# DIAGNijmegen/bodyct-dram-emph-subtype

Hardware: AMD Instinct MI355X
Metric: CT volumes/sec (train step, 1x128x256x256) (higher is better)
Workload: dtype f32; 1 GPU; BASELINE configs[1]: resnet18segcls train step (fwd+loss+bwd+Adam), batch 2/GPU, 1x128x256x256, fp32, inputs resident in HBM; global_batch=2, parallelism=dp1, hip_graph=False, streams=2

## Files before the change

### bodyct-dram-emph-subtype_amd/csrc/bn.hip

```cpp
#include <stdlib.h>
#include <atomic>
#include "common.h"

namespace {

template <typename T>
__global__ void reduce_partials_kernel(const T* __restrict__ partial, double* __restrict__ out, int nparts,
                                       int RC, double tail, int has_tail) {
  __shared__ double sm[256];
  const int col = blockIdx.x * 64 + (threadIdx.x & 63);
  const int lane4 = threadIdx.x >> 6;
  const int S = gridDim.y, sidx = blockIdx.y;
  double s = 0.0;
  if (col < RC)
    for (int p = sidx + S * lane4; p < nparts; p += 4 * S) s += (double)partial[(long)p * RC + col];
  sm[threadIdx.x] = s;
  __syncthreads();
  if (lane4 == 0 && col < RC)
    out[(long)sidx * RC + col] = sm[threadIdx.x] + sm[threadIdx.x + 64] + sm[threadIdx.x + 128] + sm[threadIdx.x + 192];
  if (has_tail && blockIdx.x == 0 && blockIdx.y == 0 && threadIdx.x == 0) out[RC] = tail;
}

__global__ void bn_finalize_kernel(const double* __restrict__ sums, double count_host,
                                   const double* __restrict__ count_dev, const float* __restrict__ gamma,
// ... 25 lines not shown
  scale[c] = sc;
  shift[c] = (float)((double)beta[c] - m * (double)gamma[c] * is);
}

struct FoldFinalize {
  double count;
  const float* gamma; const float* beta; float* rmean; float* rvar;
  float momentum, eps; int update;
  float* mean; float* invstd; float* scale; float* shift;
};
constexpr int FOLD_XMAX = 512;

__global__ __launch_bounds__(1024) void fold_partials_kernel(const float* __restrict__ partial, double* scratch,
                                                             double* __restrict__ sums, float* __restrict__ sums_f32,
                                                             float* __restrict__ f32_row1, const int nparts, const int RC,
                                                             const double tail,
                                                             const int has_tail, unsigned* __restrict__ ticket,
                                                             const FoldFinalize ff) {
  __shared__ double sm[1024];
  __shared__ double tot[64];
  __shared__ unsigned s_ticket;
  const int t64 = threadIdx.x & 63, lane4 = threadIdx.x >> 6;
  const int C = RC >> 1;
  const int col = ff.gamma ? (t64 >> 5) * C + blockIdx.x * 32 + (t64 & 31) : blockIdx.x * 64 + t64;
  const bool live = ff.gamma ? (blockIdx.x * 32 + (t64 & 31) < C) : (col < RC);
  const int S = gridDim.y, sidx = blockIdx.y;
  double s = 0.0;
  if (live) {
    const int step = 16 * S;
    int p = sidx + S * lane4;
    for (; p + 7 * step < nparts; p += 8 * step) {
      float v[8];
#pragma unroll
      for (int j = 0; j < 8; ++j) v[j] = partial[(long)(p + j * step) * RC + col];
#pragma unroll
      for (int j = 0; j < 8; ++j) s += (double)v[j];
    }
    for (; p < nparts; p += step) s += (double)partial[(long)p * RC + col];
  }
  sm[threadIdx.x] = s;
  __syncthreads();
  double total = 0.0;
  if (lane4 == 0) {
#pragma unroll
    for (int j = 0; j < 16; ++j) total += sm[t64 + 64 * j];
  }
  if (S > 1) {
    if (lane4 == 0 && live) scratch[(long)sidx * RC + col] = total;
    __threadfence();
    __syncthreads();
    if (threadIdx.x == 0) s_ticket = atomicAdd(&ticket[blockIdx.x], 1u);
    __syncthreads();
    if (s_ticket != (unsigned)S - 1) return;
    __threadfence();
    if (lane4 == 0 && live) {
      total = 0.0;
      int k = 0;
      for (; k + 8 <= S; k += 8) {
        double v[8];
#pragma unroll
        for (int j = 0; j < 8; ++j)
          v[j] = __hip_atomic_load(scratch + (long)(k + j) * RC + col, __ATOMIC_RELAXED, __HIP_MEMORY_SCOPE_AGENT);
#pragma unroll
        for (int j = 0; j < 8; ++j) total += v[j];
      }
      for (; k < S; ++k)
        total += __hip_atomic_load(scratch + (long)k * RC + col, __ATOMIC_RELAXED, __HIP_MEMORY_SCOPE_AGENT);
    }
  }
  if (lane4 == 0 && live) {
    sums[col] = total;
    if (sums_f32) {
      if (f32_row1 && col >= C) f32_row1[col - C] = (float)total;
      else sums_f32[col] = (float)total;
    }
  }
  if (has_tail && blockIdx.x == 0 && threadIdx.x == 0) sums[RC] = tail;
  if (!ff.gamma) return;
  if (lane4 == 0) tot[t64] = total;
  __syncthreads();
  const int c = blockIdx.x * 32 + threadIdx.x;
  if (threadIdx.x < 32 && c < C) {
    const double m = tot[threadIdx.x] / ff.count;
    double v = tot[32 + threadIdx.x] / ff.count - m * m;
    if (v < 0.0) v = 0.0;
    if (ff.update) {
      const double unb = ff.count > 1.0 ? v * (ff.count / (ff.count - 1.0)) : v;
      ff.rmean[c] = (float)((1.0 - (double)ff.momentum) * (double)ff.rmean[c] + (double)ff.momentum * m);
      ff.rvar[c] = (float)((1.0 - (double)ff.momentum) * (double)ff.rvar[c] + (double)ff.momentum * unb);
    }
    const double is = 1.0 / sqrt(v + (double)ff.eps);
    ff.mean[c] = (float)m;
    ff.invstd[c] = (float)is;
    ff.scale[c] = (float)((double)ff.gamma[c] * is);
    ff.shift[c] = (float)((double)ff.beta[c] - m * (double)ff.gamma[c] * is);
  }
}

template <int RES, typename T>
__global__ void bn_apply_kernel(const T* __restrict__ y, const float* __restrict__ scale,
                                const float* __restrict__ shift, const T* __restrict__ res, int Cr, int rs,
                                T* __restrict__ z, int D, int H, int W, int C, long total4, int relu) {
  const int Q = C >> 2;
  for (long i = blockIdx.x * (long)blockDim.x + threadIdx.x; i < total4; i += (long)gridDim.x * blockDim.x) {
    const int q = (int)(i % Q);
    const float4 sc = *reinterpret_cast<const float4*>(scale + 4 * q);
// ... 359 lines not shown
  }
  const long t0 = n4 * 4;
  for (long i = t0 + blockIdx.x * (long)blockDim.x + threadIdx.x; i < n; i += (long)gridDim.x * blockDim.x)
    os[i] = as[i] + bs[i];
}

inline int ew_grid(long total4) {
  long b = (total4 + 255) / 256;
  return (int)(b > 4096 ? 4096 : (b < 1 ? 1 : b));
}

inline int rows_per_block(long long rows) {
  long long rpb = (rows + 1023) / 1024;
  if (rpb < 64) rpb = 64;
  return (int)rpb;
}

}

extern "C" int dram_reduce_partials_stages(int nparts) {
  if (nparts <= 64) return 1;
  int s = (nparts + 31) / 32;
  return s > 64 ? 64 : s;
}

extern "C" int dram_reduce_partials(const float* partial, double* sums, double* scratch, int nparts, int R, int C,
                                    double tail, int has_tail, dram_stream_t stream) {
  if (!partial || !sums || nparts < 1 || R < 1 || C < 1) return DRAM_ERR_BAD_ARG;
  const int RC = R * C;
  const int S = dram_reduce_partials_stages(nparts);
  hipStream_t st = (hipStream_t)stream;
  DramProf prof(DRAM_FAM_BN, 0, 0.0, 4.0 * (double)nparts * RC + 8.0 * RC, st);
  if (S == 1) {
    hipLaunchKernelGGL((reduce_partials_kernel<float>), dim3((RC + 63) / 64, 1), dim3(256), 0, st, partial, sums,
                       nparts, RC, tail, has_tail);
  } else {
    if (!scratch) return DRAM_ERR_WORKSPACE;
    hipLaunchKernelGGL((reduce_partials_kernel<float>), dim3((RC + 63) / 64, S), dim3(256), 0, st, partial, scratch,
                       nparts, RC, 0.0, 0);
    DRAM_LAUNCH_CHECK();
    hipLaunchKernelGGL((reduce_partials_kernel<double>), dim3((RC + 63) / 64, 1), dim3(256), 0, st,
                       (const double*)scratch, sums, S, RC, tail, has_tail);
  }
  DRAM_LAUNCH_CHECK();
  return DRAM_OK;
}

extern "C" int dram_fold_partials_stages(int nparts) {
  if (nparts <= 1024) return 1;
  const int s = (nparts + 511) / 512;
  return s > 64 ? 64 : s;
}

static int fold_launch(const float* partial, double* sums, double* scratch, float* sums_f32, float* f32_row1, int nparts,
                       int RC, double tail, int has_tail, const FoldFinalize& ff, hipStream_t st) {
  const int S = dram_fold_partials_stages(nparts);
  const int gx = ff.gamma ? (RC / 2 + 31) / 32 : (RC + 63) / 64;
  if (S > 1 && gx > FOLD_XMAX) return DRAM_ERR_UNSUPPORTED;
  unsigned* ticket = nullptr;
  if (S > 1) {
    ticket = reinterpret_cast<unsigned*>(scratch + (long)S * RC);
    const hipError_t e = hipMemsetAsync(ticket, 0, sizeof(unsigned) * gx, st);
    if (e != hipSuccess) return (int)e;
  }
  DramProf prof(DRAM_FAM_BN, 0, 0.0, 4.0 * (double)nparts * RC + 8.0 * RC, st);
  hipLaunchKernelGGL(fold_partials_kernel, dim3(gx, S), dim3(1024), 0, st, partial, scratch, sums, sums_f32, f32_row1,
                     nparts, RC, tail, has_tail, ticket, ff);
  DRAM_LAUNCH_CHECK();
  return DRAM_OK;
}

extern "C" int dram_fold_partials(const float* partial, double* sums, double* scratch, float* sums_f32, float* f32_row1,
                                  int nparts, int R, int C, double tail, int has_tail, dram_stream_t stream) {
  if (!partial || !sums || !scratch || nparts < 1 || R < 1 || C < 1) return DRAM_ERR_BAD_ARG;
  if (f32_row1 && (R != 2 || !sums_f32)) return DRAM_ERR_BAD_ARG;
  FoldFinalize ff{};
  return fold_launch(partial, sums, scratch, sums_f32, f32_row1, nparts, R * C, tail, has_tail, ff, (hipStream_t)stream);
}

extern "C" int dram_bn_fold_finalize(const float* partial, double* sums, double* scratch, int nparts, int C, double count,
                                     const float* gamma, const float* beta, float* running_mean, float* running_var,
                                     float momentum, float eps, int update_running, float* mean, float* invstd,
                                     float* scale, float* shift, dram_stream_t stream) {
  if (!partial || !sums || !scratch || nparts < 1 || C < 1 || count <= 0.0) return DRAM_ERR_BAD_ARG;
  if (!gamma || !beta || !mean || !invstd || !scale || !shift) return DRAM_ERR_BAD_ARG;
  if (update_running && (!running_mean || !running_var)) return DRAM_ERR_BAD_ARG;
  FoldFinalize ff{count, gamma, beta, running_mean, running_var, momentum, eps, update_running, mean, invstd, scale, shift};
  return fold_launch(partial, sums, scratch, nullptr, nullptr, nparts, 2 * C, 0.0, 0, ff, (hipStream_t)stream);
}

extern "C" int dram_bn_finalize(const double* sums, double count, const double* count_dev, const float* gamma,
                                const float* beta,
                                float* running_mean, float* running_var, float momentum, float eps,
                                int update_running, float* mean, float* invstd, float* scale, float* shift, int C,
                                dram_stream_t stream) {
  if (!gamma || !beta || !mean || !invstd || !scale || !shift || C < 1) return DRAM_ERR_BAD_ARG;
  if (!sums && (!running_mean || !running_var)) return DRAM_ERR_BAD_ARG;
  if (sums && !count_dev && count <= 0.0) return DRAM_ERR_BAD_ARG;
  if (update_running && (!running_mean || !running_var)) return DRAM_ERR_BAD_ARG;
  DramProf prof(DRAM_FAM_BN, 1, 0.0, 4.0 * 10.0 * C, (hipStream_t)stream);
  hipLaunchKernelGGL(bn_finalize_kernel, dim3((C + 255) / 256), dim3(256), 0, (hipStream_t)stream, sums, count,
                     count_dev, gamma, beta, running_mean, running_var, momentum, eps, update_running, mean, invstd, scale,
                     shift, C);
  DRAM_LAUNCH_CHECK();
  return DRAM_OK;
}

template <typename T>
static int bn_apply_impl(const T* y, const float* scale, const float* shift, const T* residual, int Dr, int Hr, int Wr,
                         int Cr, int rs, T* z, int B, int D, int H, int W, int C, int relu, dram_stream_t stream) {
  if (!y || !scale || !shift || !z || B < 1 || D < 1 || H < 1 || W < 1 || C < 4 || (C & 3)) return DRAM_ERR_BAD_ARG;
  const long total4 = (long)B * D * H * W * (C >> 2);
  hipStream_t s = (hipStream_t)stream;
  const int grid = ew_blocks(total4, 256);
  const double res_frac = !residual ? 0.0 : ((double)Cr / C) / ((double)rs * rs * rs);
  DramProf prof(DRAM_FAM_BN, 2, 0.0, 4.0 * sizeof(T) * (double)total4 * (2.0 + res_frac), s);
  const int Q = C >> 2;
  const bool identity = residual && rs == 1 && Cr == C && Dr == D && Hr == H && Wr == W;
  if ((!residual || identity) && 256 % Q == 0) {
    const int g1 = ew_blocks(total4, 1024);
#define BN_SHOT_(RES_, NT_) hipLaunchKernelGGL((bn_apply_shot_kernel<RES_, T, NT_>), dim3(g1), dim3(256), 0, s, y, scale, \
                                               shift, residual, z, Q, total4, relu)
    const bool nt = ew_stream(sizeof(T) * 4 * total4);
    if (!residual) { if (nt) BN_SHOT_(0, true); else BN_SHOT_(0, false); }
    else           { if (nt) BN_SHOT_(1, true); else BN_SHOT_(1, false); }
#undef BN_SHOT_
  } else if (!residual) {
    hipLaunchKernelGGL((bn_apply_kernel<0, T>), dim3(grid), dim3(256), 0, s, y, scale, shift, (const T*)nullptr, 0,
                       1, z, D, H, W, C, total4, relu);
  } else if (identity) {
    hipLaunchKernelGGL((bn_apply_kernel<1, T>), dim3(grid), dim3(256), 0, s, y, scale, shift, residual,
                       Cr, 1, z, D, H, W, C, total4, relu);
  } else {
    if ((Cr & 3) || Cr < 4 || Cr > C || rs < 1) return DRAM_ERR_BAD_ARG;
    if ((D - 1) * rs >= Dr || (H - 1) * rs >= Hr || (W - 1) * rs >= Wr) return DRAM_ERR_BAD_ARG;
    hipLaunchKernelGGL((bn_apply_shortcut_a_kernel<T>), dim3(grid), dim3(256), 0, s, y, scale, shift,
                       residual, Dr, Hr, Wr, Cr, rs, z, D, H, W, C, total4, relu);
  }
  DRAM_LAUNCH_CHECK();
  return DRAM_OK;
}
// ... 151 lines not shown
```

### bodyct-dram-emph-subtype_amd/csrc/pool_up.hip

```cpp
#include <stdlib.h>
#include <initializer_list>
#include "common.h"

namespace {

inline int ew_grid(long total) { return ew_blocks(total, 256); }

template <typename T, int VW>
__global__ void maxpool_fwd_kernel(const T* __restrict__ x, T* __restrict__ y,
                                   uint8_t* __restrict__ amax, int D, int H, int W, int C, int Do, int Ho, int Wo,
                                   long total) {
  const int Q = C / VW;
  for (long i = blockIdx.x * (long)blockDim.x + threadIdx.x; i < total; i += (long)gridDim.x * blockDim.x) {
    const int q = (int)(i % Q);
    long v = i / Q;
    const int xo = (int)(v % Wo); v /= Wo;
    const int yo = (int)(v % Ho); v /= Ho;
    const int zo = (int)(v % Do);
    const long b = v / Do;
    fvec<VW> m;
    int am[VW];
#pragma unroll
    for (int k = 0; k < VW; ++k) { m.v[k] = -INFINITY; am[k] = 0; }
    bool first = true;
// ... 258 lines not shown
      o.v[k] += w_ * t.x; o.v[k + 1] += w_ * t.y; o.v[k + 2] += w_ * t.z; o.v[k + 3] += w_ * t.w; \
    }                                                                                        \
  }
      UPT_ACC(za, ya, xa, wz0 * wy0 * wx0) UPT_ACC(za, ya, xc, wz0 * wy0 * wx1)
      UPT_ACC(za, yc, xa, wz0 * wy1 * wx0) UPT_ACC(za, yc, xc, wz0 * wy1 * wx1)
      UPT_ACC(zc, ya, xa, wz1 * wy0 * wx0) UPT_ACC(zc, ya, xc, wz1 * wy0 * wx1)
      UPT_ACC(zc, yc, xa, wz1 * wy1 * wx0) UPT_ACC(zc, yc, xc, wz1 * wy1 * wx1)
#undef UPT_ACC
      const long vox = ((b * Do + zo) * Ho + yo) * (long)Wo + xo;
      stv<T, VW>(cat, vox * Ct + cb + VW * q, o);
    }
  }
  for (int e = tid; e < 512 * Qk; e += 256) {
    const int qq = e % Qk, v = e / Qk;
    const int zo = z0 + (v >> 6), yo = y0 + ((v >> 3) & 7), xo = x0 + (v & 7);
    if (zo >= Do || yo >= Ho || xo >= Wo) continue;
    const long vox = ((b * Do + zo) * Ho + yo) * (long)Wo + xo;
    stv<T, VW>(cat, vox * Ct + Cu + VW * qq,
               ldv<T, VW>(skip, (((b * Dk + zo + oz) * Hk + yo + oy) * Wk + xo + ox) * (long)Ck + VW * qq));
  }
}

__device__ __forceinline__ void dst_range(int s, float scale, int out, int& lo, int& hi) {
  if (scale <= 0.f) { lo = 0; hi = out - 1; return; }
  const float inv = 1.f / scale;
  lo = (int)floorf((float)(s - 1) * inv) - 1;
  hi = (int)ceilf((float)(s + 1) * inv) + 1;
  if (lo < 0) lo = 0;
  if (hi > out - 1) hi = out - 1;
}

struct UpAxis {
  int lo;
  float w[6];
};
__device__ __forceinline__ UpAxis up_axis(int s, float scale, int in, int out) {
  UpAxis t;
  int lo = scale > 0.f ? (int)floorf((float)(s - 1) / scale) - 1 : 0;
  if (lo < 0) lo = 0;
  t.lo = lo;
#pragma unroll
  for (int j = 0; j < 6; ++j) {
    const int d = lo + j;
    int a0, a1;
    float u0, u1;
    lin_src(d, scale, in, a0, a1, u0, u1);
    const float w = (a0 == s ? u0 : 0.f) + (a1 == s ? u1 : 0.f);
    t.w[j] = d < out ? w : 0.f;
  }
  return t;
}

template <typename T, int VW>
__global__ void upcat_bwd_src_kernel(const T* __restrict__ dcat, T* __restrict__ dsrc, int Ds, int Hs, int Ws,
                                     int Cu, int Ct, float sz, float sy, float sx, long total) {
  const int Do = 2 * Ds, Ho = 2 * Hs, Wo = 2 * Ws;
  const int Qu = Cu / VW;
  for (long i = blockIdx.x * (long)blockDim.x + threadIdx.x; i < total; i += (long)gridDim.x * blockDim.x) {
    const int q = (int)(i % Qu);
    long v = i / Qu;
    const int xs = (int)(v % Ws); v /= Ws;
    const int ys = (int)(v % Hs); v /= Hs;
    const int zs = (int)(v % Ds);
    const long b = v / Ds;
    const UpAxis tz = up_axis(zs, sz, Ds, Do), ty = up_axis(ys, sy, Hs, Ho), tx = up_axis(xs, sx, Ws, Wo);
    fvec<VW> acc;
#pragma unroll
    for (int k = 0; k < VW; ++k) acc.v[k] = 0.f;
#pragma unroll
    for (int jz = 0; jz < 6; ++jz) {
      if (tz.w[jz] == 0.f) continue;
#pragma unroll
      for (int jy = 0; jy < 6; ++jy) {
        const float wzy = tz.w[jz] * ty.w[jy];
        if (wzy == 0.f) continue;
        const T* row = dcat + (((b * Do + tz.lo + jz) * Ho + ty.lo + jy) * (long)Wo + tx.lo) * (long)Ct + VW * q;
        fvec<VW> g[6];
#pragma unroll
        for (int jx = 0; jx < 6; ++jx)
          g[jx] = ldv<T, VW>(row, (long)(tx.w[jx] != 0.f ? jx : 0) * Ct);
#pragma unroll
        for (int jx = 0; jx < 6; ++jx) {
          const float w_ = wzy * tx.w[jx];
#pragma unroll
          for (int k = 0; k < VW; ++k) acc.v[k] = __builtin_fmaf(w_, g[jx].v[k], acc.v[k]);
        }
      }
    }
    stv<T, VW>(dsrc, VW * i, acc);
  }
}

template <typename T, int VW>
__global__ void upcat_bwd_skip_kernel(const T* __restrict__ dcat, T* __restrict__ dskip, int Do, int Ho,
                                      int Wo, int Cu, int Dk, int Hk, int Wk, int Ck, int oz, int oy, int ox,
                                      long total) {
  const int Qk = Ck / VW;
  const int Ct = Cu + Ck;
  for (long i = blockIdx.x * (long)blockDim.x + threadIdx.x; i < total; i += (long)gridDim.x * blockDim.x) {
    const int q = (int)(i % Qk);
    long v = i / Qk;
    const int xk = (int)(v % Wk); v /= Wk;
    const int yk = (int)(v % Hk); v /= Hk;
    const int zk = (int)(v % Dk);
    const long b = v / Dk;
    const int zo = zk - oz, yo = yk - oy, xo = xk - ox;
    fvec<VW> o;
#pragma unroll
    for (int k = 0; k < VW; ++k) o.v[k] = 0.f;
    if (zo >= 0 && zo < Do && yo >= 0 && yo < Ho && xo >= 0 && xo < Wo)
      o = ldv<T, VW>(dcat, (((b * Do + zo) * Ho + yo) * Wo + xo) * (long)Ct + Cu + VW * q);
    stv<T, VW>(dskip, VW * i, o);
  }
}

__global__ __launch_bounds__(256) void upproject_kernel(const float* __restrict__ dense, const float* __restrict__ ess,
                                                        float* __restrict__ out, float* __restrict__ partial, int D,
                                                        int H, int W, int Do, int Ho, int Wo, float sz, float sy,
                                                        float sx, long vps, int nblk) {
  __shared__ float sm[4];
  const int b = blockIdx.y;
  float s = 0.f;
  for (long v = blockIdx.x * (long)blockDim.x + threadIdx.x; v < vps; v += (long)gridDim.x * blockDim.x) {
    long r = v;
    const int xo = (int)(r % Wo); r /= Wo;
    const int yo = (int)(r % Ho);
    const int zo = (int)(r / Ho);
    int z0, z1, y0, y1, x0, x1;
    float wz0, wz1, wy0, wy1, wx0, wx1;
    lin_src(zo, sz, D, z0, z1, wz0, wz1);
    lin_src(yo, sy, H, y0, y1, wy0, wy1);
    lin_src(xo, sx, W, x0, x1, wx0, wx1);
    const float* p = dense + (long)b * D * H * W;
#define DV(zz, yy, xx) p[((long)(zz) * H + (yy)) * W + (xx)]
    const float val = wz0 * (wy0 * (wx0 * DV(z0, y0, x0) + wx1 * DV(z0, y0, x1)) + wy1 * (wx0 * DV(z0, y1, x0) + wx1 * DV(z0, y1, x1))) +
                      wz1 * (wy0 * (wx0 * DV(z1, y0, x0) + wx1 * DV(z1, y0, x1)) + wy1 * (wx0 * DV(z1, y1, x0) + wx1 * DV(z1, y1, x1)));
#undef DV
    const float o = val * ess[(long)b * vps + v];
    out[(long)b * vps + v] = o;
    s += o;
  }
  s = wave_sum(s);
  if ((threadIdx.x & 63) == 0) sm[threadIdx.x >> 6] = s;
// ... 91 lines not shown
extern "C" int dram_maxpool_bwd_bf16(const void* dy, const uint8_t* argmax, const void* add, int add_stride, void* dx,
                                     int B, int D, int H, int W, int C, dram_stream_t stream) {
  return maxpool_bwd_impl<bf16_t>((const bf16_t*)dy, argmax, (const bf16_t*)add, add_stride, (bf16_t*)dx, B, D, H, W, C,
                                  stream);
}

template <typename T>
static int upcat_fwd_impl(const T* src, const T* skip, T* cat, int B, int Ds, int Hs, int Ws, int Cu, int Dk, int Hk,
                          int Wk, int Ck, dram_stream_t stream) {
  if (!src || !cat || B < 1 || Cu < 4 || (Cu & 3) || (skip ? (Ck < 4 || (Ck & 3)) : Ck != 0)) return DRAM_ERR_BAD_ARG;
  const int Do = 2 * Ds, Ho = 2 * Hs, Wo = 2 * Ws;
  if (Dk < Do || Hk < Ho || Wk < Wo) return DRAM_ERR_BAD_ARG;
  const int oz = (Dk - Do + 1) / 2, oy = (Hk - Ho + 1) / 2, ox = (Wk - Wo + 1) / 2;
  const long total4 = (long)B * Do * Ho * Wo * ((Cu + Ck) >> 2);
  const long tiles = (long)B * ((Do + 7) / 8) * ((Ho + 7) / 8) * ((Wo + 7) / 8);
  DramProf prof(DRAM_FAM_POOL_UP, 2, 0.0,
                (double)sizeof(T) * ((double)B * Ds * Hs * Ws * Cu + (double)B * Do * Ho * Wo * Ck + 4.0 * total4),
                (hipStream_t)stream);
  const bool wide = pool_wide(sizeof(T), {Cu, Ck});
  if (Cu % 64 == 0 && tiles >= 512 && tiles < (1L << 31) && !tune_env("DRAM_UPCAT_UNTILED")) {
    POOL_LAUNCH(wide, upcat_fwd_tiled_kernel, (unsigned)tiles, src, skip, cat, Ds, Hs, Ws, Cu, Dk, Hk, Wk, Ck, oz, oy, ox,
                ac_scale(Ds, Do), ac_scale(Hs, Ho), ac_scale(Ws, Wo), (Do + 7) / 8, (Ho + 7) / 8, (Wo + 7) / 8);
    DRAM_LAUNCH_CHECK();
    return DRAM_OK;
  }
  const long total = wide ? total4 / 2 : total4;
  POOL_LAUNCH(wide, upcat_fwd_kernel, ew_grid(total), src, skip, cat, Ds, Hs, Ws, Cu, Dk, Hk, Wk, Ck, oz, oy, ox,
              ac_scale(Ds, Do), ac_scale(Hs, Ho), ac_scale(Ws, Wo), total);
  DRAM_LAUNCH_CHECK();
  return DRAM_OK;
}
extern "C" int dram_upcat_fwd(const float* src, const float* skip, float* cat, int B, int Ds, int Hs, int Ws, int Cu,
                              int Dk, int Hk, int Wk, int Ck, dram_stream_t stream) {
  return upcat_fwd_impl<float>(src, skip, cat, B, Ds, Hs, Ws, Cu, Dk, Hk, Wk, Ck, stream);
}
extern "C" int dram_upcat_fwd_bf16(const void* src, const void* skip, void* cat, int B, int Ds, int Hs, int Ws, int Cu,
                                   int Dk, int Hk, int Wk, int Ck, dram_stream_t stream) {
  return upcat_fwd_impl<bf16_t>((const bf16_t*)src, (const bf16_t*)skip, (bf16_t*)cat, B, Ds, Hs, Ws, Cu, Dk, Hk, Wk, Ck,
                                stream);
}

template <typename T>
static int upcat_bwd_impl(const T* dcat, T* dsrc, T* dskip, int B, int Ds, int Hs, int Ws, int Cu, int Dk, int Hk, int Wk,
                          int Ck, dram_stream_t stream) {
  if (!dcat || (!dsrc && !dskip) || B < 1 || Cu < 4 || Ck < 4 || (Cu & 3) || (Ck & 3)) return DRAM_ERR_BAD_ARG;
  const int Do = 2 * Ds, Ho = 2 * Hs, Wo = 2 * Ws;
  if (Dk < Do || Hk < Ho || Wk < Wo) return DRAM_ERR_BAD_ARG;
  const int oz = (Dk - Do + 1) / 2, oy = (Hk - Ho + 1) / 2, ox = (Wk - Wo + 1) / 2;
  hipStream_t s = (hipStream_t)stream;
  const bool wide = pool_wide(sizeof(T), {Cu, Ck});
  if (dsrc) {
    const long total4 = (long)B * Ds * Hs * Ws * (Cu >> 2);
    DramProf prof(DRAM_FAM_POOL_UP, 3, 0.0, (double)sizeof(T) * ((double)B * Do * Ho * Wo * Cu + 4.0 * total4), s);
    const long total = wide ? total4 / 2 : total4;
    POOL_LAUNCH(wide, upcat_bwd_src_kernel, ew_grid(total), dcat, dsrc, Ds, Hs, Ws, Cu, Cu + Ck, ac_scale(Ds, Do),
                ac_scale(Hs, Ho), ac_scale(Ws, Wo), total);
    DRAM_LAUNCH_CHECK();
  }
  if (dskip) {
    const long total4 = (long)B * Dk * Hk * Wk * (Ck >> 2);
    DramProf prof(DRAM_FAM_POOL_UP, 4, 0.0, (double)sizeof(T) * ((double)B * Do * Ho * Wo * Ck + 4.0 * total4), s);
    const long total = wide ? total4 / 2 : total4;
    POOL_LAUNCH(wide, upcat_bwd_skip_kernel, ew_grid(total), dcat, dskip, Do, Ho, Wo, Cu, Dk, Hk, Wk, Ck, oz, oy, ox,
                total);
    DRAM_LAUNCH_CHECK();
  }
  return DRAM_OK;
}
extern "C" int dram_upcat_bwd(const float* dcat, float* dsrc, float* dskip, int B, int Ds, int Hs, int Ws, int Cu,
                              int Dk, int Hk, int Wk, int Ck, dram_stream_t stream) {
  return upcat_bwd_impl<float>(dcat, dsrc, dskip, B, Ds, Hs, Ws, Cu, Dk, Hk, Wk, Ck, stream);
}
extern "C" int dram_upcat_bwd_bf16(const void* dcat, void* dsrc, void* dskip, int B, int Ds, int Hs, int Ws, int Cu,
                                   int Dk, int Hk, int Wk, int Ck, dram_stream_t stream) {
  return upcat_bwd_impl<bf16_t>((const bf16_t*)dcat, (bf16_t*)dsrc, (bf16_t*)dskip, B, Ds, Hs, Ws, Cu, Dk, Hk, Wk, Ck,
                                stream);
}

extern "C" int dram_upproject_nblk(long long vps) {
  long long b = (vps + 1023) / 1024;
  return (int)(b > 1024 ? 1024 : (b < 1 ? 1 : b));
}

extern "C" int dram_upproject(const float* dense, const float* ess, float* out, float* partial, int B, int D, int H,
                              int W, int Do, int Ho, int Wo, dram_stream_t stream) {
  if (!dense || !ess || !out || !partial || B < 1 || D < 1 || H < 1 || W < 1 || Do < 1 || Ho < 1 || Wo < 1)
    return DRAM_ERR_BAD_ARG;
  const long vps = (long)Do * Ho * Wo;
  const int nblk = dram_upproject_nblk(vps);
  DramProf prof(DRAM_FAM_POOL_UP, 5, 0.0, 4.0 * ((double)B * D * H * W + 2.0 * B * (double)vps), (hipStream_t)stream);
  hipLaunchKernelGGL(upproject_kernel, dim3(nblk, B), dim3(256), 0, (hipStream_t)stream, dense, ess, out, partial, D, H,
                     W, Do, Ho, Wo, ac_scale(D, Do), ac_scale(H, Ho), ac_scale(W, Wo), vps, nblk);
  DRAM_LAUNCH_CHECK();
  return DRAM_OK;
}
```

### bodyct-dram-emph-subtype_amd/ops.py

```python
from __future__ import annotations

import contextlib
import ctypes
import math
import os
import threading
import weakref
from dataclasses import dataclass
from typing import Dict, List, Optional, Tuple

import torch

from . import _lib
from ._lib import DramConvDesc

Tensor = torch.Tensor


def _L():
    return _lib.load()


_TLS = threading.local()

# ... 742 lines not shown
def stem_fwd(x: Tensor, w: Tensor, want_stats: bool, out_dtype=torch.float32):
    _req(x, "x")
    if x.dim() != 4:
        raise ValueError("stem_fwd: x must be [B,D,H,W]")
    _req(w, "w", shape=(64, 1, 7, 7, 7))
    B, D, H, W = x.shape
    Do, Ho, Wo = stem_out(D), stem_out(H), stem_out(W)
    if out_dtype not in (torch.float32, BF16):
        raise TypeError(f"stem_fwd: unsupported storage type {out_dtype}")
    y = torch.empty((B, Do, Ho, Wo, 64), device=x.device, dtype=out_dtype)
    stats = None
    if want_stats:
        nt = _L().dram_stem_num_tiles(B, Do, Ho, Wo)
        stats = torch.empty((nt, 2, 64), device=x.device, dtype=torch.float32)
    with _span("stem_fwd_kernel", 2.0 * B * Do * Ho * Wo * 64 * 343):
        sfx = "" if out_dtype != BF16 else ("_bf16mm" if tuning_env("DRAM_STEM_BF16", "1") != "0" else "_bf16")
        _chk(_fn("dram_stem_fwd", sfx)(_p(x), _p(w), _p(y), _p(stats), B, D, H, W, _stream()), "dram_stem_fwd" + sfx)
    return y, stats


def stem_bwd_weight(x: Tensor, dy: Tensor, out: Optional[Tensor] = None) -> Tensor:
    _req(x, "x")
    B, D, H, W = x.shape
    sfx = _act(dy, "dy", (B, stem_out(D), stem_out(H), stem_out(W), 64))
    nbytes = _L().dram_stem_bwd_weight_workspace(B, D, H, W)
    ws = torch.empty(((nbytes + 3) // 4,), device=x.device, dtype=torch.float32)
    dw = out if out is not None else torch.empty((64, 1, 7, 7, 7), device=x.device, dtype=torch.float32)
    _req(dw, "dw", shape=(64, 1, 7, 7, 7))
    with _span("stem_wgrad_kernel+reduce", 2.0 * dy.numel() * 343):
        if sfx and tuning_env("DRAM_STEM_BF16", "1") != "0":
            sfx = "_bf16mm"
        _chk(_fn("dram_stem_bwd_weight", sfx)(_p(x), _p(dy), _p(dw), B, D, H, W, _p(ws), nbytes, _stream()),
             "dram_stem_bwd_weight" + sfx)
    return dw


def stem_bwd_data(dy: Tensor, w: Tensor, in_shape) -> Tensor:
    B, D, H, W = (int(v) for v in in_shape)
    if min(B, D, H, W) < 1:
        raise ValueError(f"stem_bwd_data: bad input shape {tuple(in_shape)}")
    sfx = _act(dy, "dy", (B, stem_out(D), stem_out(H), stem_out(W), 64))
    _req(w, "w", shape=(64, 1, 7, 7, 7))
    nbytes = _L().dram_stem_bwd_data_workspace(B, D, H, W)
    ws = torch.empty(((nbytes + 3) // 4,), device=dy.device, dtype=torch.float32)
    dx = torch.empty((B, D, H, W), device=dy.device, dtype=torch.float32)
    with _span("stem_dgrad_kernel+fold", 2.0 * dy.numel() * 343):
        _chk(_fn("dram_stem_bwd_data", sfx)(_p(dy), _p(w), _p(dx), B, D, H, W, _p(ws), nbytes, _stream()),
             "dram_stem_bwd_data" + sfx)
    return dx


FOLD_TICKET_DOUBLES = _lib.DRAM_FOLD_TICKET_DOUBLES


def reduce_partials(partial: Tensor, tail: Optional[float] = None, want_f32: bool = False):
    _req(partial, "partial")
    Pn, R, C = partial.shape
    stages = _L().dram_fold_partials_stages(Pn)
    n = R * C + (1 if tail is not None else 0)
    buf = torch.empty((n + stages * R * C + (FOLD_TICKET_DOUBLES if stages > 1 else 0),), device=partial.device,
                      dtype=torch.float64)
    flat = buf[:n]
    f32 = [torch.empty((C,), device=partial.device, dtype=torch.float32) for _ in range(R)] if want_f32 else None
    if want_f32 and R > 2:
        raise ValueError("reduce_partials: the float copy supports at most two rows")
    _chk(_L().dram_fold_partials(_p(partial), _p(flat), _p(buf[n:]), _p(f32[0]) if f32 else None,
                                 _p(f32[1]) if (f32 and R == 2) else None, Pn, R, C,
                                 float(tail) if tail is not None else 0.0, int(tail is not None), _stream()),
         "dram_fold_partials")
    res = (flat, flat[:R * C].view(R, C)) if tail is not None else (flat.view(R, C),)
    if want_f32:
        res = res + (f32,)
    return res if len(res) > 1 else res[0]


def bn_fold_finalize(partial: Tensor, count: float, gamma: Tensor, beta: Tensor, running_mean: Tensor,
                     running_var: Tensor, momentum: float, eps: float):
    _req(partial, "partial")
    Pn, R, C = partial.shape
    if R != 2:
        raise ValueError("bn_fold_finalize: expected [P,2,C] partial sums")
    for t, nm in ((gamma, "gamma"), (beta, "beta"), (running_mean, "running_mean"), (running_var, "running_var")):
        _req(t, nm, shape=(C,))
    stages = _L().dram_fold_partials_stages(Pn)
    buf = torch.empty(((1 + stages) * 2 * C + (FOLD_TICKET_DOUBLES if stages > 1 else 0),), device=partial.device,
                      dtype=torch.float64)
    out = torch.empty((4, C), device=partial.device, dtype=torch.float32)
    _chk(_L().dram_bn_fold_finalize(_p(partial), _p(buf), _p(buf[2 * C:]), Pn, C, float(count), _p(gamma), _p(beta),
                                    _p(running_mean), _p(running_var), float(momentum), float(eps), 1, _p(out[0]),
                                    _p(out[1]), _p(out[2]), _p(out[3]), _stream()), "dram_bn_fold_finalize")
    return out[0], out[1], out[2], out[3]


def bn_finalize(sums: Optional[Tensor], count: float, gamma: Tensor, beta: Tensor, running_mean: Tensor,
                running_var: Tensor, momentum: float, eps: float, update_running: bool,
                count_dev: Optional[Tensor] = None):
    C = gamma.numel()
    if count_dev is not None:
        _req(count_dev, "count_dev", dtype=torch.float64, shape=(1,))
    _req(gamma, "gamma", shape=(C,))
    _req(beta, "beta", shape=(C,))
    _req(running_mean, "running_mean", shape=(C,))
    _req(running_var, "running_var", shape=(C,))
    if sums is not None:
        _req(sums, "sums", dtype=torch.float64, shape=(2, C))
    out = torch.empty((4, C), device=gamma.device, dtype=torch.float32)
    mean, invstd, scale, shift = out[0], out[1], out[2], out[3]
    _chk(_L().dram_bn_finalize(_p(sums), float(count), _p(count_dev), _p(gamma), _p(beta), _p(running_mean), _p(running_var),
                               float(momentum), float(eps), int(update_running), _p(mean), _p(invstd), _p(scale),
                               _p(shift), C, _stream()), "dram_bn_finalize")
    return mean, invstd, scale, shift


def bn_apply(y: Tensor, scale: Tensor, shift: Tensor, residual: Optional[Tensor], rs: int, relu: bool) -> Tensor:
    sfx = _act(y, "y")
    B, D, H, W, C = y.shape
    _req(scale, "scale", shape=(C,))
    _req(shift, "shift", shape=(C,))
    Dr = Hr = Wr = Cr = 0
    if residual is not None:
        _act(residual, "residual", like=y)
        if residual.shape[0] != B:
            raise ValueError("bn_apply: residual batch mismatch")
        _, Dr, Hr, Wr, Cr = residual.shape
        if Cr > C or (D - 1) * rs >= Dr or (H - 1) * rs >= Hr or (W - 1) * rs >= Wr:
            raise ValueError(f"bn_apply: residual {tuple(residual.shape)} incompatible with {tuple(y.shape)} rs={rs}")
        if ((Dr - 1) // rs + 1, (Hr - 1) // rs + 1, (Wr - 1) // rs + 1) != (D, H, W):
            raise ValueError("bn_apply: strided residual does not match the output grid")
    z = torch.empty_like(y)
    _chk(_fn("dram_bn_apply", sfx)(_p(y), _p(scale), _p(shift), _p(residual), Dr, Hr, Wr, Cr, rs, _p(z), B, D, H, W, C,
                                   int(relu), _stream()), "dram_bn_apply")
    return z


def _rows(t: Tensor) -> int:
    return t.numel() // t.shape[-1]


def _mask_args(z, y, scale, shift, relu):
    C = y.shape[-1]
    if relu and z is not None:
# ... 729 lines not shown
```

### include/dram_hip.h

```cpp
#ifndef DRAM_HIP_H
#define DRAM_HIP_H

#include <stddef.h>
#include <stdint.h>

#ifdef __cplusplus
extern "C" {
#endif

typedef void* dram_stream_t;

#define DRAM_OK 0
#define DRAM_ERR_BAD_ARG (-1)
#define DRAM_ERR_UNSUPPORTED (-2)
#define DRAM_ERR_WORKSPACE (-3)

#define DRAM_ABI_VERSION 7
int dram_version(void);
const char* dram_build_info(void);
const char* dram_abi_hash(void);
unsigned long long dram_stream_capture_id(dram_stream_t stream);

enum {
  DRAM_FAM_CONV_WINO2D = 0,
// ... 76 lines not shown
int dram_wino_conv3d_fwd_bn(const float* x_pre, const float* pscale, const float* pshift, const float* uf, const float* bias,
                            float* y, float* stats_partial, float* v_keep, const DramConvDesc* d, void* workspace,
                            size_t workspace_bytes, dram_stream_t stream);
int dram_wino_conv3d_bwd_data(const float* dy, const float* ub, float* dx, const float* add,
                              const float* gate, const DramConvDesc* desc, void* workspace,
                              size_t workspace_bytes, dram_stream_t stream);
int dram_wino_num_stat_rows_bwd(const DramConvDesc* desc);
int dram_wino_conv3d_bwd_data_bn(const float* dy, const float* ub, float* dx, const float* bn_y, const float* bn_mean,
                                 const float* bn_invstd, const float* bn_scale, const float* bn_shift,
                                 float* stats_partial, const DramConvDesc* desc, void* workspace, size_t workspace_bytes,
                                 dram_stream_t stream);
int dram_wino_conv3d_bwd_weight(const float* x, const float* v_cache, const float* dy, float* dw,
                                const DramConvDesc* desc, void* workspace, size_t workspace_bytes,
                                dram_stream_t stream);

int dram_wino2d_applicable(const DramConvDesc* desc);
int dram_wino2d_num_stat_rows(const DramConvDesc* desc);
int dram_wino2d_pack_weight(const float* w, float* uf, float* ub, int Cout, int Cin, dram_stream_t stream);
int dram_wino2d_conv3d_fwd(const float* x, const float* uf, const float* bias, float* y,
                           float* stats_partial, const DramConvDesc* desc, dram_stream_t stream);
int dram_wino2d_conv3d_bwd_data(const float* dy, const float* ub, float* dx, const float* add,
                                const float* gate, const DramConvDesc* desc, dram_stream_t stream);

int dram_wgrad_w2d_applicable(const DramConvDesc* desc);
size_t dram_wgrad_w2d_workspace(const DramConvDesc* desc);
int dram_wgrad_w2d(const float* x, const float* dy, float* dw, const DramConvDesc* desc, void* workspace,
                   size_t workspace_bytes, dram_stream_t stream);

int dram_conv1x1_applicable(const DramConvDesc* desc);
int dram_conv1x1_num_stat_rows(const DramConvDesc* desc);
int dram_conv1x1_fwd(const float* x, const float* w2d, const float* bias, float* y, float* stats_partial,
                     const DramConvDesc* desc, dram_stream_t stream);
int dram_conv1x1_bwd_data(const float* dy, const float* wt, float* dx, const float* add, const float* gate,
                          const DramConvDesc* desc, dram_stream_t stream);
size_t dram_conv1x1_bwd_weight_workspace(const DramConvDesc* desc);
int dram_conv1x1_bwd_weight(const float* x, const float* dy, float* dw, const DramConvDesc* desc, void* workspace,
                            size_t workspace_bytes, dram_stream_t stream);

int dram_conv_algo(const DramConvDesc* desc);

int dram_stem_num_tiles(int B, int Do, int Ho, int Wo);
int dram_stem_fwd(const float* x, const float* w, float* y, float* stats_partial, int B, int D, int H,
                  int W, dram_stream_t stream);
size_t dram_stem_bwd_weight_workspace(int B, int D, int H, int W);
int dram_stem_bwd_weight(const float* x, const float* dy, float* dw, int B, int D, int H, int W,
                         void* workspace, size_t workspace_bytes, dram_stream_t stream);
size_t dram_stem_bwd_data_workspace(int B, int D, int H, int W);
int dram_stem_bwd_data(const float* dy, const float* w, float* dx, int B, int D, int H, int W, void* workspace,
                       size_t workspace_bytes, dram_stream_t stream);

int dram_reduce_partials_stages(int nparts);
#define DRAM_FOLD_TICKET_DOUBLES 256
int dram_fold_partials_stages(int nparts);
int dram_fold_partials(const float* partial, double* sums, double* scratch, float* sums_f32, float* f32_row1, int nparts,
                       int R, int C, double tail, int has_tail, dram_stream_t stream);
int dram_bn_fold_finalize(const float* partial, double* sums, double* scratch, int nparts, int C, double count,
                          const float* gamma, const float* beta, float* running_mean, float* running_var, float momentum,
                          float eps, int update_running, float* mean, float* invstd, float* scale, float* shift,
                          dram_stream_t stream);
int dram_reduce_partials(const float* partial, double* sums, double* scratch, int nparts, int R, int C,
                         double tail, int has_tail, dram_stream_t stream);

int dram_bn_finalize(const double* sums, double count, const double* count_dev, const float* gamma, const float* beta,
                     float* running_mean, float* running_var, float momentum, float eps,
                     int update_running, float* mean, float* invstd, float* scale, float* shift,
                     int C, dram_stream_t stream);

int dram_bn_apply(const float* y, const float* scale, const float* shift, const float* residual,
                  int Dr, int Hr, int Wr, int Cr, int rs, float* z, int B, int D, int H, int W, int C,
                  int relu, dram_stream_t stream);

int dram_colsum_nparts(long long rows, int C);
int dram_bn_bwd_reduce(const float* dz, const float* z, const float* y, const float* mean,
                       const float* invstd, const float* scale, const float* shift, float* partial,
                       long long rows, int C, int relu, dram_stream_t stream);
int dram_bn_bwd_apply_nparts(long long rows, int C);
int dram_bn_bwd_apply(const float* dz, const float* z, const float* y, const float* mean,
                      const float* invstd, const float* gamma, const float* scale, const float* shift,
                      const double* sums, double count, const double* count_dev, float* dy,
                      float* colsum_partial, long long rows, int C, int relu, dram_stream_t stream);
int dram_bn_bwd_apply_eval(const float* dz, const float* z, const float* y, const float* scale, const float* shift,
                           float* dy, float* colsum_partial, long long rows, int C, int relu, dram_stream_t stream);
int dram_colsum(const float* a, float* partial, long long rows, int C, dram_stream_t stream);

int dram_maxpool_fwd(const float* x, float* y, uint8_t* argmax, int B, int D, int H, int W, int C,
                     dram_stream_t stream);
int dram_bn_maxpool_fwd(const float* y, const float* scale, const float* shift, float* z, float* pooled, uint8_t* argmax,
                        int B, int D, int H, int W, int C, dram_stream_t stream);
int dram_maxpool_bwd(const float* dy, const uint8_t* argmax, const float* add, int add_stride, float* dx,
                     int B, int D, int H, int W, int C, dram_stream_t stream);

int dram_upcat_fwd(const float* src, const float* skip, float* cat, int B, int Ds, int Hs, int Ws, int Cu,
                   int Dk, int Hk, int Wk, int Ck, dram_stream_t stream);
int dram_upcat_bwd(const float* dcat, float* dsrc, float* dskip, int B, int Ds, int Hs, int Ws, int Cu,
                   int Dk, int Hk, int Wk, int Ck, dram_stream_t stream);

int dram_upmix_stat_rows(long long nvox);
int dram_upmix_axis_fwd(const void* in, int in_bf16, float* out, long long outer, int Ni, int m, int C,
                        dram_stream_t stream);
int dram_upmix_axis_fwd_final(const float* in, const void* base, void* out, int out_bf16, float* stats, long long outer,
                              int Ni, int m, int C, dram_stream_t stream);
int dram_upmix_axis_bwd(const void* g, int g_bf16, void* h, int h_bf16, long long outer, int Ni, int m, int C,
                        dram_stream_t stream);
int dram_upmix_split_weight(const float* w, float* wlo, float* ws, int Co, int Cu, int Cs, dram_stream_t stream);
int dram_upmix_merge_wgrad(const float* dwlo, const float* dws, float* dw, int Co, int Cu, int Cs, dram_stream_t stream);

int dram_head_nblk(long long voxels_per_sample);
int dram_head_fwd(const float* x, const float* w, const float* bias, const float* lungs, int Dl, int Hl,
                  int Wl, float* dense, float* partial, int B, int D, int H, int W, int NO, int sigmoid,
// ... 227 lines not shown
```

Baseline: 55.33 volumes/sec.

## Tile upsample-concat backward through LDS and drop per-call ticket memsets

Adds an LDS-tiled upcat backward-to-source kernel. Each block stages a halo tile of the upsampled gradient once, and its threads gather their trilinear weights from shared memory instead of reloading overlapping global rows. It falls back to the global gather when a footprint leaves the tile. Separately, the BN fold reduction now uses a persistent per-stream ticket buffer that the last block resets itself, removing a hipMemsetAsync before every multi-stage fold. This adds a per-stream or per-capture ticket cache and new LDS-size attribute setup, and it changes the ABI signatures.

```diff
diff --git a/bodyct-dram-emph-subtype_amd/csrc/bn.hip b/bodyct-dram-emph-subtype_amd/csrc/bn.hip
--- a/bodyct-dram-emph-subtype_amd/csrc/bn.hip
+++ b/bodyct-dram-emph-subtype_amd/csrc/bn.hip
@@ -101,6 +101,7 @@
     if (threadIdx.x == 0) s_ticket = atomicAdd(&ticket[blockIdx.x], 1u);
     __syncthreads();
     if (s_ticket != (unsigned)S - 1) return;
+    if (threadIdx.x == 0) __hip_atomic_store(&ticket[blockIdx.x], 0u, __ATOMIC_RELAXED, __HIP_MEMORY_SCOPE_AGENT);
     __threadfence();
     if (lane4 == 0 && live) {
       total = 0.0;
@@ -566,17 +567,13 @@
   return s > 64 ? 64 : s;
 }
 
-static int fold_launch(const float* partial, double* sums, double* scratch, float* sums_f32, float* f32_row1, int nparts,
-                       int RC, double tail, int has_tail, const FoldFinalize& ff, hipStream_t st) {
+static int fold_launch(const float* partial, double* sums, double* scratch, unsigned* ticket, float* sums_f32,
+                       float* f32_row1, int nparts, int RC, double tail, int has_tail, const FoldFinalize& ff,
+                       hipStream_t st) {
   const int S = dram_fold_partials_stages(nparts);
   const int gx = ff.gamma ? (RC / 2 + 31) / 32 : (RC + 63) / 64;
   if (S > 1 && gx > FOLD_XMAX) return DRAM_ERR_UNSUPPORTED;
-  unsigned* ticket = nullptr;
-  if (S > 1) {
-    ticket = reinterpret_cast<unsigned*>(scratch + (long)S * RC);
-    const hipError_t e = hipMemsetAsync(ticket, 0, sizeof(unsigned) * gx, st);
-    if (e != hipSuccess) return (int)e;
-  }
+  if (S > 1 && !ticket) return DRAM_ERR_WORKSPACE;
   DramProf prof(DRAM_FAM_BN, 0, 0.0, 4.0 * (double)nparts * RC + 8.0 * RC, st);
   hipLaunchKernelGGL(fold_partials_kernel, dim3(gx, S), dim3(1024), 0, st, partial, scratch, sums, sums_f32, f32_row1,
                      nparts, RC, tail, has_tail, ticket, ff);
@@ -584,15 +581,18 @@
   return DRAM_OK;
 }
 
-extern "C" int dram_fold_partials(const float* partial, double* sums, double* scratch, float* sums_f32, float* f32_row1,
-                                  int nparts, int R, int C, double tail, int has_tail, dram_stream_t stream) {
+extern "C" int dram_fold_partials(const float* partial, double* sums, double* scratch, void* ticket, float* sums_f32,
+                                  float* f32_row1, int nparts, int R, int C, double tail, int has_tail,
+                                  dram_stream_t stream) {
   if (!partial || !sums || !scratch || nparts < 1 || R < 1 || C < 1) return DRAM_ERR_BAD_ARG;
   if (f32_row1 && (R != 2 || !sums_f32)) return DRAM_ERR_BAD_ARG;
   FoldFinalize ff{};
-  return fold_launch(partial, sums, scratch, sums_f32, f32_row1, nparts, R * C, tail, has_tail, ff, (hipStream_t)stream);
-}
-
-extern "C" int dram_bn_fold_finalize(const float* partial, double* sums, double* scratch, int nparts, int C, double count,
+  return fold_launch(partial, sums, scratch, (unsigned*)ticket, sums_f32, f32_row1, nparts, R * C, tail, has_tail, ff,
+                     (hipStream_t)stream);
+}
+
+extern "C" int dram_bn_fold_finalize(const float* partial, double* sums, double* scratch, void* ticket, int nparts,
+                                     int C, double count,
                                      const float* gamma, const float* beta, float* running_mean, float* running_var,
                                      float momentum, float eps, int update_running, float* mean, float* invstd,
                                      float* scale, float* shift, dram_stream_t stream) {
@@ -600,7 +600,8 @@
   if (!gamma || !beta || !mean || !invstd || !scale || !shift) return DRAM_ERR_BAD_ARG;
   if (update_running && (!running_mean || !running_var)) return DRAM_ERR_BAD_ARG;
   FoldFinalize ff{count, gamma, beta, running_mean, running_var, momentum, eps, update_running, mean, invstd, scale, shift};
-  return fold_launch(partial, sums, scratch, nullptr, nullptr, nparts, 2 * C, 0.0, 0, ff, (hipStream_t)stream);
+  return fold_launch(partial, sums, scratch, (unsigned*)ticket, nullptr, nullptr, nparts, 2 * C, 0.0, 0, ff,
+                     (hipStream_t)stream);
 }
 
 extern "C" int dram_bn_finalize(const double* sums, double count, const double* count_dev, const float* gamma,
diff --git a/bodyct-dram-emph-subtype_amd/csrc/pool_up.hip b/bodyct-dram-emph-subtype_amd/csrc/pool_up.hip
--- a/bodyct-dram-emph-subtype_amd/csrc/pool_up.hip
+++ b/bodyct-dram-emph-subtype_amd/csrc/pool_up.hip
@@ -334,6 +334,36 @@
 }
 
 template <typename T, int VW>
+__device__ __forceinline__ fvec<VW> upcat_bwd_src_gather(const T* __restrict__ dcat, long b, const UpAxis& tz,
+                                                         const UpAxis& ty, const UpAxis& tx, int Do, int Ho, int Wo,
+                                                         int Ct, int coff) {
+  fvec<VW> acc;
+#pragma unroll
+  for (int k = 0; k < VW; ++k) acc.v[k] = 0.f;
+#pragma unroll
+  for (int jz = 0; jz < 6; ++jz) {
+    if (tz.w[jz] == 0.f) continue;
+#pragma unroll
+    for (int jy = 0; jy < 6; ++jy) {
+      const float wzy = tz.w[jz] * ty.w[jy];
+      if (wzy == 0.f) continue;
+      const T* row = dcat + (((b * Do + tz.lo + jz) * Ho + ty.lo + jy) * (long)Wo + tx.lo) * (long)Ct + coff;
+      fvec<VW> g[6];
+#pragma unroll
+      for (int jx = 0; jx < 6; ++jx)
+        g[jx] = ldv<T, VW>(row, (long)(tx.w[jx] != 0.f ? jx : 0) * Ct);
+#pragma unroll
+      for (int jx = 0; jx < 6; ++jx) {
+        const float w_ = wzy * tx.w[jx];
+#pragma unroll
+        for (int k = 0; k < VW; ++k) acc.v[k] = __builtin_fmaf(w_, g[jx].v[k], acc.v[k]);
+      }
+    }
+  }
+  return acc;
+}
+
+template <typename T, int VW>
 __global__ void upcat_bwd_src_kernel(const T* __restrict__ dcat, T* __restrict__ dsrc, int Ds, int Hs, int Ws,
                                      int Cu, int Ct, float sz, float sy, float sx, long total) {
   const int Do = 2 * Ds, Ho = 2 * Hs, Wo = 2 * Ws;
@@ -346,9 +376,87 @@
     const int zs = (int)(v % Ds);
     const long b = v / Ds;
     const UpAxis tz = up_axis(zs, sz, Ds, Do), ty = up_axis(ys, sy, Hs, Ho), tx = up_axis(xs, sx, Ws, Wo);
-    fvec<VW> acc;
-#pragma unroll
-    for (int k = 0; k < VW; ++k) acc.v[k] = 0.f;
+    stv<T, VW>(dsrc, VW * i, upcat_bwd_src_gather<T, VW>(dcat, b, tz, ty, tx, Do, Ho, Wo, Ct, VW * q));
+  }
+}
+
+constexpr int UBZ = 2, UBY = 4, UBX = 4;
+constexpr int UTZ = 2 * UBZ + 2, UTY = 2 * UBY + 2, UTX = 2 * UBX + 2;
+constexpr int UTV = UTZ * UTY * UTX;
+
+__device__ __forceinline__ int up_tile_origin(int s0, float scale) {
+  const int t = (int)floorf((float)(s0 - 1) / scale) + 1;
+  return t < 0 ? 0 : t;
+}
+__device__ __forceinline__ bool up_tile_fits(const UpAxis& t, int origin, int extent) {
+  bool ok = true;
+#pragma unroll
+  for (int j = 0; j < 6; ++j) {
+    const int rel = t.lo + j - origin;
+    ok &= (t.w[j] == 0.f) | ((rel >= 0) & (rel < extent));
+  }
+  return ok;
+}
+
+template <int QS>
+__global__ __launch_bounds__(32 * QS, 4) void upcat_bwd_src_tiled_kernel(
+    const float* __restrict__ dcat, float* __restrict__ dsrc, int Ds, int Hs, int Ws, int Cu, int Ct, float sz, float sy,
+    float sx, int nslab, int nbz, int nby, int nbx, int nblk) {
+  extern __shared__ __attribute__((aligned(16))) float4 tile[];
+  const int Do = 2 * Ds, Ho = 2 * Hs, Wo = 2 * Ws;
+  int r = xcd_remap(blockIdx.x, nblk);
+  const int slab = r % nslab; r /= nslab;
+  const int bz = r % nbz; r /= nbz;
+  const int bx = r % nbx; r /= nbx;
+  const int by = r % nby;
+  const long b = r / nby;
+  const int z0 = bz * UBZ, y0 = by * UBY, x0 = bx * UBX, c0 = slab * (4 * QS);
+  const int oz = __builtin_amdgcn_readfirstlane(up_tile_origin(z0, sz)),
+            oy = __builtin_amdgcn_readfirstlane(up_tile_origin(y0, sy)),
+            ox = __builtin_amdgcn_readfirstlane(up_tile_origin(x0, sx));
+  const int tid = threadIdx.x;
+  const int q = tid % QS, v = tid / QS;
+  constexpr int RPI = 32 / UTX, IT = (UTZ * UTY + RPI - 1) / RPI;
+  static_assert(RPI * IT == UTZ * UTY, "whole rows per iteration");
+  if (v < RPI * UTX) {
+    const char* base = reinterpret_cast<const char*>(dcat + b * ((long)Do * Ho * Wo * Ct) + c0);
+    const int lx = v % UTX, r0 = v / UTX;
+    const unsigned xoff = (unsigned)(min(ox + lx, Wo - 1) * Ct + 4 * q) * 4u, rowb = (unsigned)(Wo * Ct) * 4u;
+    float4 st[IT];
+#pragma unroll
+    for (int i = 0; i < IT; ++i) {
+      int lz = (RPI * i) / UTY, ly = (RPI * i) % UTY + r0;
+      if ((RPI * i) % UTY + RPI - 1 >= UTY && ly >= UTY) { ly -= UTY; lz += 1; }
+      const int zc = min(oz + lz, Do - 1), yc = min(oy + ly, Ho - 1);
+      st[i] = *reinterpret_cast<const float4*>(base + ((unsigned)(zc * Ho + yc) * rowb + xoff));
+    }
+    __builtin_amdgcn_sched_barrier(0);
+    int r2 = r0;
+    asm volatile("" : "+v"(r2));
+    const bool inx = ox + lx < Wo;
+    float4* col = tile + (r2 * UTX + (lx & 1) * (UTX / 2) + (lx >> 1)) * QS + q;
+#pragma unroll
+    for (int i = 0; i < IT; ++i) {
+      int lz = (RPI * i) / UTY, ly = (RPI * i) % UTY + r2;
+      if ((RPI * i) % UTY + RPI - 1 >= UTY && ly >= UTY) { ly -= UTY; lz += 1; }
+      const float m = (inx & (oz + lz < Do) & (oy + ly < Ho)) ? 1.f : 0.f;
+      col[RPI * i * UTX * QS] = make_float4(st[i].x * m, st[i].y * m, st[i].z * m, st[i].w * m);
+    }
+  }
+  __syncthreads();
+  const int zs = z0 + v / (UBY * UBX), ys = y0 + (v / UBX) % UBY, xs = x0 + v % UBX;
+  if (zs >= Ds || ys >= Hs || xs >= Ws) return;
+  const UpAxis tz = up_axis(zs, sz, Ds, Do), ty = up_axis(ys, sy, Hs, Ho), tx = up_axis(xs, sx, Ws, Wo);
+  fvec<4> acc;
+  if (up_tile_fits(tz, oz, UTZ) & up_tile_fits(ty, oy, UTY) & up_tile_fits(tx, ox, UTX)) {
+    int xo[6];
+#pragma unroll
+    for (int jx = 0; jx < 6; ++jx) {
+      const int rel = min(max(tx.lo + jx - ox, 0), UTX - 1);
+      xo[jx] = ((rel & 1) * (UTX / 2) + (rel >> 1)) * QS + q;
+    }
+#pragma unroll
+    for (int k = 0; k < 4; ++k) acc.v[k] = 0.f;
 #pragma unroll
     for (int jz = 0; jz < 6; ++jz) {
       if (tz.w[jz] == 0.f) continue;
@@ -356,21 +464,24 @@
       for (int jy = 0; jy < 6; ++jy) {
         const float wzy = tz.w[jz] * ty.w[jy];
         if (wzy == 0.f) continue;
-        const T* row = dcat + (((b * Do + tz.lo + jz) * Ho + ty.lo + jy) * (long)Wo + tx.lo) * (long)Ct + VW * q;
-        fvec<VW> g[6];
-#pragma unroll
-        for (int jx = 0; jx < 6; ++jx)
-          g[jx] = ldv<T, VW>(row, (long)(tx.w[jx] != 0.f ? jx : 0) * Ct);
+        const float4* row = tile + ((tz.lo + jz - oz) * UTY + (ty.lo + jy - oy)) * (UTX * QS);
+        float4 g[6];
+#pragma unroll
+        for (int jx = 0; jx < 6; ++jx) g[jx] = row[xo[jx]];
 #pragma unroll
         for (int jx = 0; jx < 6; ++jx) {
           const float w_ = wzy * tx.w[jx];
-#pragma unroll
-          for (int k = 0; k < VW; ++k) acc.v[k] = __builtin_fmaf(w_, g[jx].v[k], acc.v[k]);
+          acc.v[0] = __builtin_fmaf(w_, g[jx].x, acc.v[0]);
+          acc.v[1] = __builtin_fmaf(w_, g[jx].y, acc.v[1]);
+          acc.v[2] = __builtin_fmaf(w_, g[jx].z, acc.v[2]);
+          acc.v[3] = __builtin_fmaf(w_, g[jx].w, acc.v[3]);
         }
       }
     }
-    stv<T, VW>(dsrc, VW * i, acc);
-  }
+  } else {
+    acc = upcat_bwd_src_gather<float, 4>(dcat, b, tz, ty, tx, Do, Ho, Wo, Ct, c0 + 4 * q);
+  }
+  stv<float, 4>(dsrc, ((((b * Ds + zs) * Hs + ys) * (long)Ws + xs) * (long)Cu) + c0 + 4 * q, acc);
 }
 
 template <typename T, int VW>
@@ -568,9 +679,41 @@
   if (dsrc) {
     const long total4 = (long)B * Ds * Hs * Ws * (Cu >> 2);
     DramProf prof(DRAM_FAM_POOL_UP, 3, 0.0, (double)sizeof(T) * ((double)B * Do * Ho * Wo * Cu + 4.0 * total4), s);
-    const long total = wide ? total4 / 2 : total4;
-    POOL_LAUNCH(wide, upcat_bwd_src_kernel, ew_grid(total), dcat, dsrc, Ds, Hs, Ws, Cu, Cu + Ck, ac_scale(Ds, Do),
-                ac_scale(Hs, Ho), ac_scale(Ws, Wo), total);
+    const int nbz = (Ds + UBZ - 1) / UBZ, nby = (Hs + UBY - 1) / UBY, nbx = (Ws + UBX - 1) / UBX;
+    const int qu = Cu >> 2, qs = qu % 8 == 0 ? 8 : (qu % 4 == 0 ? 4 : (qu % 2 == 0 ? 2 : 1));
+    const long nblk = (long)B * nbz * nby * nbx * (qu / qs);
+    bool tiled = false;
+    if constexpr (sizeof(T) == 4) {
+      tiled = Ds >= UBZ && Hs >= UBY && Ws >= UBX && Dk == Do && Hk == Ho && Wk == Wo && nblk < (1L << 31) &&
+              (long)Do * Ho * Wo * (Cu + Ck) < (1L << 30);
+      if (tiled) {
+#define UP_TILED_(QS_)                                                                                               \
+  do {                                                                                                               \
+     \
+    static bool lds_set[64] = {};                                                                                    \
+    int dev = 0;                                                                                                     \
+    if (UTV * QS_ * 16 > (64 << 10) && hipGetDevice(&dev) == hipSuccess && dev >= 0 && dev < 64 && !lds_set[dev]) {  \
+      const hipError_t e = hipFuncSetAttribute(reinterpret_cast<const void*>(&upcat_bwd_src_tiled_kernel<QS_>),      \
+                                               hipFuncAttributeMaxDynamicSharedMemorySize, UTV * QS_ * 16);          \
+      if (e != hipSuccess) return (int)e;                                                                            \
+      lds_set[dev] = true;                                                                                           \
+    }                                                                                                                \
+    hipLaunchKernelGGL((upcat_bwd_src_tiled_kernel<QS_>), dim3((unsigned)nblk), dim3(32 * QS_), UTV * QS_ * 16, s,   \
+                       dcat, dsrc, Ds, Hs, Ws, Cu, Cu + Ck, ac_scale(Ds, Do), ac_scale(Hs, Ho), ac_scale(Ws, Wo),     \
+                       qu / qs, nbz, nby, nbx, (int)nblk);                                                           \
+  } while (0)
+        if (qs == 8) UP_TILED_(8);
+        else if (qs == 4) UP_TILED_(4);
+        else if (qs == 2) UP_TILED_(2);
+        else UP_TILED_(1);
+#undef UP_TILED_
+      }
+    }
+    if (!tiled) {
+      const long total = wide ? total4 / 2 : total4;
+      POOL_LAUNCH(wide, upcat_bwd_src_kernel, ew_grid(total), dcat, dsrc, Ds, Hs, Ws, Cu, Cu + Ck, ac_scale(Ds, Do),
+                  ac_scale(Hs, Ho), ac_scale(Ws, Wo), total);
+    }
     DRAM_LAUNCH_CHECK();
   }
   if (dskip) {
diff --git a/bodyct-dram-emph-subtype_amd/ops.py b/bodyct-dram-emph-subtype_amd/ops.py
--- a/bodyct-dram-emph-subtype_amd/ops.py
+++ b/bodyct-dram-emph-subtype_amd/ops.py
@@ -818,19 +818,43 @@
 
 FOLD_TICKET_DOUBLES = _lib.DRAM_FOLD_TICKET_DOUBLES
 
+_FOLD_TICKETS: Dict[tuple, Tensor] = {}
+_CAPTURE_TICKETS: Dict[tuple, "weakref.ref"] = {}
+
+
+def _fold_tickets(device) -> Tensor:
+    device = torch.device(device)
+    cid = capture_id()
+    if cid:
+        key = (device, _stream().value, cid)
+        ref = _CAPTURE_TICKETS.get(key)
+        t = ref() if ref is not None else None
+        if t is None:
+            t = torch.zeros((FOLD_TICKET_DOUBLES,), device=device, dtype=torch.float64)
+            _keep_for_capture(t)
+            for k in [k for k, r in _CAPTURE_TICKETS.items() if r() is None]:
+                del _CAPTURE_TICKETS[k]
+            _CAPTURE_TICKETS[key] = weakref.ref(t)
+        return t
+    key = (device, _stream().value)
+    t = _FOLD_TICKETS.get(key)
+    if t is None:
+        t = _FOLD_TICKETS[key] = torch.zeros((FOLD_TICKET_DOUBLES,), device=device, dtype=torch.float64)
+    return t
+
 
 def reduce_partials(partial: Tensor, tail: Optional[float] = None, want_f32: bool = False):
     _req(partial, "partial")
     Pn, R, C = partial.shape
     stages = _L().dram_fold_partials_stages(Pn)
     n = R * C + (1 if tail is not None else 0)
-    buf = torch.empty((n + stages * R * C + (FOLD_TICKET_DOUBLES if stages > 1 else 0),), device=partial.device,
-                      dtype=torch.float64)
+    buf = torch.empty((n + stages * R * C,), device=partial.device, dtype=torch.float64)
+    tickets = _fold_tickets(partial.device) if stages > 1 else None
     flat = buf[:n]
     f32 = [torch.empty((C,), device=partial.device, dtype=torch.float32) for _ in range(R)] if want_f32 else None
     if want_f32 and R > 2:
         raise ValueError("reduce_partials: the float copy supports at most two rows")
-    _chk(_L().dram_fold_partials(_p(partial), _p(flat), _p(buf[n:]), _p(f32[0]) if f32 else None,
+    _chk(_L().dram_fold_partials(_p(partial), _p(flat), _p(buf[n:]), _p(tickets), _p(f32[0]) if f32 else None,
                                  _p(f32[1]) if (f32 and R == 2) else None, Pn, R, C,
                                  float(tail) if tail is not None else 0.0, int(tail is not None), _stream()),
          "dram_fold_partials")
@@ -849,10 +873,11 @@
     for t, nm in ((gamma, "gamma"), (beta, "beta"), (running_mean, "running_mean"), (running_var, "running_var")):
         _req(t, nm, shape=(C,))
     stages = _L().dram_fold_partials_stages(Pn)
-    buf = torch.empty(((1 + stages) * 2 * C + (FOLD_TICKET_DOUBLES if stages > 1 else 0),), device=partial.device,
-                      dtype=torch.float64)
+    buf = torch.empty(((1 + stages) * 2 * C,), device=partial.device, dtype=torch.float64)
+    tickets = _fold_tickets(partial.device) if stages > 1 else None
     out = torch.empty((4, C), device=partial.device, dtype=torch.float32)
-    _chk(_L().dram_bn_fold_finalize(_p(partial), _p(buf), _p(buf[2 * C:]), Pn, C, float(count), _p(gamma), _p(beta),
+    _chk(_L().dram_bn_fold_finalize(_p(partial), _p(buf), _p(buf[2 * C:]), _p(tickets), Pn, C, float(count), _p(gamma),
+                                    _p(beta),
                                     _p(running_mean), _p(running_var), float(momentum), float(eps), 1, _p(out[0]),
                                     _p(out[1]), _p(out[2]), _p(out[3]), _stream()), "dram_bn_fold_finalize")
     return out[0], out[1], out[2], out[3]
diff --git a/include/dram_hip.h b/include/dram_hip.h
--- a/include/dram_hip.h
+++ b/include/dram_hip.h
@@ -152,9 +152,9 @@
 int dram_reduce_partials_stages(int nparts);
 #define DRAM_FOLD_TICKET_DOUBLES 256
 int dram_fold_partials_stages(int nparts);
-int dram_fold_partials(const float* partial, double* sums, double* scratch, float* sums_f32, float* f32_row1, int nparts,
-                       int R, int C, double tail, int has_tail, dram_stream_t stream);
-int dram_bn_fold_finalize(const float* partial, double* sums, double* scratch, int nparts, int C, double count,
+int dram_fold_partials(const float* partial, double* sums, double* scratch, void* ticket, float* sums_f32, float* f32_row1,
+                       int nparts, int R, int C, double tail, int has_tail, dram_stream_t stream);
+int dram_bn_fold_finalize(const float* partial, double* sums, double* scratch, void* ticket, int nparts, int C, double count,
                           const float* gamma, const float* beta, float* running_mean, float* running_var, float momentum,
                           float eps, int update_running, float* mean, float* invstd, float* scale, float* shift,
                           dram_stream_t stream);
```

After: 55.34 volumes/sec (median of 3 runs). About the same (+0.0%).
